# terryye/cuda_FlashAttention

Measured on AMD Instinct MI355X. Metric: FA2 fwd+bwd TFLOP/s at (B=4,H=16,N=8192,d=128); % MFMA peak, higher is better.
Workload: dtype bf16; 1 GPU; FA2 forward+backward bf16, (B=4,H=16,N=8192,d=128) per GPU, non-causal (BASELINE configs[2]); flops = 14 B H N^2 d; B=4, H=16, N=8192, d=128, parallelism=head-sharded replicas x1

## Files before the change

### cuda_flashattention_amd/csrc/fa2_bwd_bf16.hip

```cpp
#include <type_traits>

#include "fa2_regfile.h"
#include "fa2_launch.h"

namespace fa2 {

constexpr float kNoKeyRC = -1.0e30f;
constexpr float kNoKeyLq = 1.0e30f;

template <int D>
__global__ void __launch_bounds__(256) fa2_bwd_delta_kernel(const __bf16* __restrict__ dO,
                                                            const __bf16* __restrict__ O,
                                                            const float* __restrict__ L,
                                                            float* __restrict__ Dv, float* __restrict__ RC,
                                                            size_t rows, int nq, int q_hs, int q_row0, size_t rc_plane,
                                                            float inv_scale)
{
    const size_t r = ((size_t)blockIdx.x * 256 + threadIdx.x) >> 4;
    const int sub = threadIdx.x & 15;
    const size_t head = r / (size_t)nq, i = r % (size_t)nq;
    const size_t row = head * (size_t)q_hs + i;
    const size_t prow = row + (size_t)q_row0;
    float acc = 0.0f;
    if (r < rows) {
#pragma unroll
        for (int c = sub * 8; c < D; c += 128) {
            const bf16x8 a = *reinterpret_cast<const bf16x8*>(dO + row * D + c);
            const bf16x8 b = *reinterpret_cast<const bf16x8*>(O + row * D + c);
#pragma unroll
            for (int e = 0; e < 8; ++e) acc += (float)a[e] * (float)b[e];
        }
    }
#pragma unroll
    for (int off = 8; off >= 1; off >>= 1) acc += __shfl_xor(acc, off, 16);
    if (r < rows && sub == 0) {
        Dv[prow] = acc;
        const float l = L[row];
        RC[prow] = l == -INFINITY ? kNoKeyRC : -l * inv_scale;
        RC[rc_plane + prow] = -acc;
    }
}

__global__ void __launch_bounds__(256) fa2_bwd_dsink_kernel(const float* __restrict__ Dv, const float* __restrict__ L,
                                                            const float* __restrict__ sink, float* __restrict__ dsink,
                                                            int batch, int heads, int nq, int q_hs, int q_row0)
{
    __shared__ float part[256];
    const int h = blockIdx.x, tid = threadIdx.x;
    const float s = sink[h];
    float acc = 0.0f;
    if (s != -INFINITY) {
        for (int b = 0; b < batch; ++b) {
            const size_t row0 = ((size_t)b * heads + h) * (size_t)q_hs;
#pragma unroll 8
            for (int i = tid; i < nq; i += 256)
                acc -= __builtin_amdgcn_exp2f((s - L[row0 + i]) * kLog2e) * Dv[row0 + q_row0 + i];
        }
    }
    part[tid] = acc;
    __syncthreads();
#pragma unroll
    for (int off = 128; off >= 1; off >>= 1) {
        if (tid < off) part[tid] += part[tid + off];
        __syncthreads();
    }
    if (tid == 0) dsink[h] = part[0];
}

static hipError_t launch_dsink(const SinkGrad& sg, const BwdArgs& a, int nq, hipStream_t stream)
{
    if (!sg.sink || !sg.dsink || sg.heads < 1 || a.BH % sg.heads != 0) return hipErrorInvalidValue;
    hipLaunchKernelGGL(fa2_bwd_dsink_kernel, dim3((unsigned)sg.heads), dim3(256), 0, stream, (const float*)a.D, a.L, sg.sink, sg.dsink,
                       a.BH / sg.heads, sg.heads, nq, a.q_hs, a.q_row0);
    return hipGetLastError();
}

constexpr int kBwdRows = 256;
constexpr int kDqWaves = 4;
constexpr int kDqKV = 64;
constexpr int kDkQ = 32;

typedef __attribute__((address_space(3))) void* lptr_t;

#include "fa2_bwd_dq_body.inc"

#define FA2_DQ_CLOBBERS "memory", "vcc", FA2_RF512
#define FA2_DQ_OPS_128 [r0] "v"(roff[0]), [r1] "v"(roff[1]), [r2] "v"(roff[2]), [r3] "v"(roff[3]), [r4] "v"(roff[4]), [r5] "v"(roff[5]), \
    [r6] "v"(roff[6]), [r7] "v"(roff[7]), [t0] "v"(toff[0]), [t1] "v"(toff[1]), [t2] "v"(toff[2]), [t3] "v"(toff[3]), [t4] "v"(toff[4]),     \
    [t5] "v"(toff[5]), [t6] "v"(toff[6]), [t7] "v"(toff[7])
#define FA2_DQ_OPS_64 [r0] "v"(roff[0]), [r1] "v"(roff[1]), [r2] "v"(roff[2]), [r3] "v"(roff[3]), [t0] "v"(toff[0]), [t1] "v"(toff[1]),    \
    [t2] "v"(toff[2]), [t3] "v"(toff[3])
// ... 382 lines not shown
        tile(std::integral_constant<int, 1>{}, t + 1);
    }
    }

    asm volatile("s_waitcnt lgkmcnt(0)" ::: "memory");
    mfma_acc_settle();
    static_for<2>([&](auto KB) {
        constexpr int kb = decltype(KB)::value;
        const int key = kw0 + 32 * kb + ki;
        char* dKk = (char*)p.dK + slab + (size_t)(key < N ? key : 0) * ROWB;
        char* dVk = (char*)p.dV + slab + (size_t)(key < N ? key : 0) * ROWB;
        static_for<4 * DT>([&](auto G) {
            constexpr int dt = decltype(G)::value / 4, g = decltype(G)::value % 4;
            constexpr int RK = A_DK + 16 * (kb * DT + dt) + 4 * g, RV = A_DV + 16 * (kb * DT + dt) + 4 * g;
            bf16x4 a, b;
            a[0] = (__bf16)(aread<RK>() * p.scale); a[1] = (__bf16)(aread<RK + 1>() * p.scale);
            a[2] = (__bf16)(aread<RK + 2>() * p.scale); a[3] = (__bf16)(aread<RK + 3>() * p.scale);
            b[0] = (__bf16)aread<RV>(); b[1] = (__bf16)aread<RV + 1>();
            b[2] = (__bf16)aread<RV + 2>(); b[3] = (__bf16)aread<RV + 3>();
            if (key < N) {
                *reinterpret_cast<bf16x4*>(dKk + 2 * (32 * dt + 8 * g + 4 * h)) = a;
                *reinterpret_cast<bf16x4*>(dVk + 2 * (32 * dt + 8 * g + 4 * h)) = b;
            }
        });
    });
}

template <int D, bool CAUSAL>
__global__ void __launch_bounds__(256, 1) __attribute__((amdgpu_num_vgpr(60))) fa2_bwd_dkdv_kernel(BwdArgs p)
{
    const int ncb = (p.Nk + kDkKeys - 1) / kDkKeys;
    int kvhead, cb;
    map_block(blockIdx.x, p.BH / p.kv_group, ncb, kvhead, cb);
    bwd_dkdv_impl<D, CAUSAL>(p, kvhead, cb);
}

template <int D, bool CAUSAL>
__global__ void __launch_bounds__(256, 1) __attribute__((amdgpu_num_vgpr(60))) fa2_bwd_dkdv_varlen_kernel(VarlenBwdArgs v)
{
    int kvhead, idx;
    map_block(blockIdx.x, v.a.BH / v.a.kv_group, v.n_key_items, kvhead, idx);
    const VarlenItem it = uniform_item(v.key_items, idx);
    bwd_dkdv_impl<D, CAUSAL>(bwd_varlen_view<D>(v.a, it), kvhead, it.block);
}

template <int D, bool CAUSAL>
static hipError_t launch_bwd_one(const BwdArgs& a, hipStream_t stream, const SinkGrad* sg)
{
    const size_t rows = (size_t)a.BH * a.Nq;
    hipError_t e = hipSuccess;
    if (a.phases & 1) {
        hipLaunchKernelGGL((fa2_bwd_delta_kernel<D>), dim3((unsigned)((rows * 16 + 255) / 256)), dim3(256), 0,
                           stream, (const __bf16*)a.dO, (const __bf16*)a.O, a.L, a.D, a.RC, rows, a.Nq, a.q_hs, a.q_row0,
                           (size_t)a.BH * a.q_hs, 1.0f / a.scale);
        e = hipGetLastError();
        if (e != hipSuccess) return e;
        if (sg && (e = launch_dsink(*sg, a, a.Nq, stream)) != hipSuccess) return e;
    }
    const int nb = (a.Nq + kBwdRows - 1) / kBwdRows;
    constexpr int lds_dq = 3 * 2 * kDqKV * D * 2;
    constexpr int lds_dk = kDkKeys * D * 2 + 2 * (2 * 2 * kDkQ * D * 2 + 512);
    if (a.phases & 2) {
        e = launch_lds<fa2_bwd_dq_kernel<D, CAUSAL>>(dim3((unsigned)(nb * a.BH)), dim3(256), lds_dq, stream, a);
        if (e != hipSuccess) return e;
    }
    if (a.phases & 4) {
        const int ncb = (a.Nk + kDkKeys - 1) / kDkKeys;
        e = launch_lds<fa2_bwd_dkdv_kernel<D, CAUSAL>>(dim3((unsigned)(ncb * (a.BH / a.kv_group))), dim3(256), lds_dk, stream, a);
    }
    return e;
}

template <int D, bool CAUSAL>
static hipError_t launch_bwd_varlen_one(const VarlenBwdArgs& v, hipStream_t stream, const SinkGrad* sg)
{
    const BwdArgs& a = v.a;
    const size_t rows = (size_t)a.BH * a.q_hs;
    hipLaunchKernelGGL((fa2_bwd_delta_kernel<D>), dim3((unsigned)((rows * 16 + 255) / 256)), dim3(256), 0, stream,
                       (const __bf16*)a.dO, (const __bf16*)a.O, a.L, a.D, a.RC, rows, a.q_hs, a.q_hs, 0, rows, 1.0f / a.scale);
    hipError_t e = hipGetLastError();
    if (e != hipSuccess) return e;
    if (sg && (e = launch_dsink(*sg, a, a.q_hs, stream)) != hipSuccess) return e;
    constexpr int lds_dq = 3 * 2 * kDqKV * D * 2;
    constexpr int lds_dk = kDkKeys * D * 2 + 2 * (2 * 2 * kDkQ * D * 2 + 512);
    e = launch_lds<fa2_bwd_dq_varlen_kernel<D, CAUSAL>>(dim3((unsigned)(v.n_row_items * a.BH)), dim3(256), lds_dq, stream, v);
    if (e != hipSuccess) return e;
    return launch_lds<fa2_bwd_dkdv_varlen_kernel<D, CAUSAL>>(dim3((unsigned)(v.n_key_items * (a.BH / a.kv_group))), dim3(256), lds_dk,
                                                            stream, v);
}

hipError_t launch_bwd_varlen_bf16(const VarlenBwdArgs& v, hipStream_t stream, const SinkGrad* sg)
{
    const BwdArgs& a = v.a;
    if (a.kv_group < 1 || a.BH % a.kv_group != 0 || v.n_row_items < 1 || v.n_key_items < 1 || !v.row_items || !v.key_items)
        return hipErrorInvalidValue;
    if (a.d == 128) return a.causal ? launch_bwd_varlen_one<128, true>(v, stream, sg) : launch_bwd_varlen_one<128, false>(v, stream, sg);
    if (a.d == 64) return a.causal ? launch_bwd_varlen_one<64, true>(v, stream, sg) : launch_bwd_varlen_one<64, false>(v, stream, sg);
    return hipErrorInvalidValue;
}

hipError_t launch_bwd_bf16(const BwdArgs& a, hipStream_t stream, const SinkGrad* sg)
{
    if (a.kv_group < 1 || a.BH % a.kv_group != 0) return hipErrorInvalidValue;
    if (a.d == 128) return a.causal ? launch_bwd_one<128, true>(a, stream, sg) : launch_bwd_one<128, false>(a, stream, sg);
    if (a.d == 64) return a.causal ? launch_bwd_one<64, true>(a, stream, sg) : launch_bwd_one<64, false>(a, stream, sg);
    return hipErrorInvalidValue;
}

}
```

### cuda_flashattention_amd/csrc/fa2_bwd_fused.hip

```cpp
#include <cstdlib>
#include <cstring>
#include <type_traits>

#include "fa2_regfile.h"
#include "fa2_launch.h"

namespace fa2 {

#include "fa2_bwd_fused_body.inc"

typedef __attribute__((address_space(3))) void* fused_lptr_t;

#ifndef FA2_FUSED_DSKEY
#define FA2_FUSED_DSKEY(row) (((row) >> 1) & 7)
#endif

#ifndef FA2_FUSED_DIAG
#define FA2_FUSED_DIAG 0
#endif

constexpr int kFusedRegFile = RF512;

#define FA2_FUSED_CLOBBERS "memory", "vcc", FA2_RF512
#define FA2_FUSED_OPS_128 [r0] "v"(roff[0]), [r1] "v"(roff[1]), [r2] "v"(roff[2]), [r3] "v"(roff[3]), [r4] "v"(roff[4]), [r5] "v"(roff[5]),  \
// ... 27 lines not shown
    FA2_FUSED_CASE(TAG, DD, 0, 0) FA2_FUSED_CASE(TAG, DD, 0, 1) FA2_FUSED_CASE(TAG, DD, 1, 0) FA2_FUSED_CASE(TAG, DD, 1, 1) FA2_FUSED_CASE(TAG, DD, 2, 0) FA2_FUSED_CASE(TAG, DD, 2, 1)
    FA2_FUSED_CASES(, 128) FA2_FUSED_CASES(64, 64)
#undef FA2_FUSED_CASES
#undef FA2_FUSED_CASE
}

template <int BUF, int PAR, int VMW>
__device__ __forceinline__ void fused_body(const uint32_t (&roff)[8], const uint32_t (&toff)[8], uint32_t rcv, float c2)
{
#define FA2_FUSED_CASE(B, P) \
    if constexpr (BUF == B && PAR == P) asm volatile(FA2_FUSED_BODY_B##B##_P##P : : FA2_FUSED_OPS_128, [vm] "i"(VMW) : FA2_FUSED_CLOBBERS);
    FA2_FUSED_CASE(0, 0) FA2_FUSED_CASE(0, 1) FA2_FUSED_CASE(1, 0) FA2_FUSED_CASE(1, 1) FA2_FUSED_CASE(2, 0) FA2_FUSED_CASE(2, 1)
#undef FA2_FUSED_CASE
}

template <int DQT>
__device__ __forceinline__ void fused_dq_atomic(__amdgpu_buffer_rsrc_t rs, uint32_t voff, uint32_t soff)
{
    asm volatile(
        "s_add_u32 s12, %2, 4096\n\ts_add_u32 s13, %2, 8192\n\ts_add_u32 s14, %2, 12288\n\t"
        "buffer_atomic_add_f32 v%c3, %0, %1, %2 offen\n\tbuffer_atomic_add_f32 v%c4, %0, %1, %2 offen offset:512\n\t"
        "buffer_atomic_add_f32 v%c5, %0, %1, %2 offen offset:1024\n\tbuffer_atomic_add_f32 v%c6, %0, %1, %2 offen offset:1536\n\t"
        "buffer_atomic_add_f32 v%c7, %0, %1, s12 offen\n\tbuffer_atomic_add_f32 v%c8, %0, %1, s12 offen offset:512\n\t"
        "buffer_atomic_add_f32 v%c9, %0, %1, s12 offen offset:1024\n\tbuffer_atomic_add_f32 v%c10, %0, %1, s12 offen offset:1536\n\t"
        "buffer_atomic_add_f32 v%c11, %0, %1, s13 offen\n\tbuffer_atomic_add_f32 v%c12, %0, %1, s13 offen offset:512\n\t"
        "buffer_atomic_add_f32 v%c13, %0, %1, s13 offen offset:1024\n\tbuffer_atomic_add_f32 v%c14, %0, %1, s13 offen offset:1536\n\t"
        "buffer_atomic_add_f32 v%c15, %0, %1, s14 offen\n\tbuffer_atomic_add_f32 v%c16, %0, %1, s14 offen offset:512\n\t"
        "buffer_atomic_add_f32 v%c17, %0, %1, s14 offen offset:1024\n\tbuffer_atomic_add_f32 v%c18, %0, %1, s14 offen offset:1536\n\t"
        "s_nop 1"
        : : "v"(voff), "s"(rs), "s"(soff), "i"(DQT), "i"(DQT + 1), "i"(DQT + 2), "i"(DQT + 3), "i"(DQT + 4), "i"(DQT + 5), "i"(DQT + 6),
            "i"(DQT + 7), "i"(DQT + 8), "i"(DQT + 9), "i"(DQT + 10), "i"(DQT + 11), "i"(DQT + 12), "i"(DQT + 13), "i"(DQT + 14),
            "i"(DQT + 15)
        : "memory", "s12", "s13", "s14", "v255");
}

template <int VF, int KS, int S>
__device__ __forceinline__ void fused_load_vfrag(const char* v0, const char* v1)
{
#ifndef FA2_FUSED_KV_NT
#define FA2_FUSED_KV_NT ""
#define FA2_FUSED_KV_AUX 0
#endif
    asm volatile("global_load_dwordx4 v[%c2:%c3], %0, off offset:%c4" FA2_FUSED_KV_NT "\n\tglobal_load_dwordx4 v[%c5:%c6], %1, off offset:%c4" FA2_FUSED_KV_NT
                 : : "v"(v0), "v"(v1), "i"(VF + 4 * S), "i"(VF + 4 * S + 3), "i"(32 * S), "i"(VF + 4 * (KS + S)), "i"(VF + 4 * (KS + S) + 3)
                 : "memory", "v255");
}

template <int DQT>
__device__ __forceinline__ void fused_dq_zero()
{
    static_for<16>([&](auto R) { vset<kFusedRegFile, CL_TOP, DQT + decltype(R)::value>(0u); });
}

constexpr int kCtlTicket = 0, kCtlNextHead = 32 * 16, kCtlError = 32 * 17, kCtlHeadmap = 32 * 18;
constexpr int kHmPad = 16;
constexpr int kSpinLimit = FA2_FUSED_SPIN_LIMIT;

struct FusedArgs {
    BwdArgs b;
    float* dQacc;
    int* ctl;
    int npad;
    const float* rc;
    int fault;
};

#ifdef FA2_TEST_HOOKS
static int g_hook_fault = 0, g_hook_grid = 0, g_hook_last_grid = 0;
extern "C" void fa2_test_set_fused_hooks(int fault, int grid) { g_hook_fault = fault; g_hook_grid = grid; }
extern "C" int fa2_test_last_fused_grid(void) { return g_hook_last_grid; }
#define FA2_HOOK_NOTE_GRID(n) (g_hook_last_grid = (n))
#else
constexpr int g_hook_fault = 0, g_hook_grid = 0;
#define FA2_HOOK_NOTE_GRID(n) ((void)0)
#endif

__device__ __forceinline__ int fused_ctl_ints(int BH, int ncb) { return kCtlHeadmap + 16 * (BH + kHmPad) + 9 * BH * ncb; }

__device__ __forceinline__ int fused_load_sc1(const int* p)
{
    int v;
    asm volatile("global_load_dword %0, %1, off sc1\n\ts_waitcnt vmcnt(0)" : "=v"(v) : "v"(p) : "memory");
    return v;
}
__device__ __forceinline__ void fused_seen_set(int v)
{
    asm volatile("v_mov_b32 v39, %0" : : "s"(v) : "v39");
}

__device__ __forceinline__ int fused_lane_id() { return (int)__builtin_amdgcn_mbcnt_hi(~0u, __builtin_amdgcn_mbcnt_lo(~0u, 0u)); }
template <int OFF>
__device__ __forceinline__ int fused_mail_read(uint32_t lds_addr)
{
    int v;
    asm volatile("v_mov_b32 %0, %1\n\tds_read_b32 %0, %0 offset:%c2\n\ts_waitcnt lgkmcnt(0)" : "=&v"(v) : "s"(lds_addr), "i"(OFF) : "memory");
    return __builtin_amdgcn_readfirstlane(v);
}

__device__ __forceinline__ void fused_store_flag(int* p, int v)
{
    asm volatile("global_store_dword %0, %1, off" : : "v"(p), "v"(v) : "memory");
}

__device__ __forceinline__ bool fused_spin_over(int* ctl, int spins)
{
    if (spins > kSpinLimit) {
        atomicExch(ctl + kCtlError, 1);
        return true;
    }
    return (spins & 1023) == 0 && fused_load_sc1(ctl + kCtlError) != 0;
}

template <bool CHAIN, bool CAUSAL, bool RAGGED = false, bool RECT = false, int HD = 128>
__global__ void __launch_bounds__(256, 1) __attribute__((amdgpu_num_vgpr(39))) fa2_bwd_fused_kernel(FusedArgs fp)
{
    static_assert(CHAIN || !RAGGED, "the atomics form has no ragged variant");
    static_assert(!RECT || (CHAIN && !CAUSAL && !RAGGED), "rectangular blocks: chained, unmasked, aligned");
    static_assert(HD == 128 || (HD == 64 && CHAIN && !RECT), "head_dim 64: chained, square");
    extern __shared__ __attribute__((aligned(16))) char smem[];
    const BwdArgs& p = fp.b;
    constexpr int D = HD, ROWB = 2 * D, KS = D / 16, DT = D / 32;
    constexpr int DQW = 128;
    constexpr int TROWS = 32;
    constexpr bool W = D == 128;
    constexpr int QRING = W ? FA2_FUSED_QRING : FA2_FUSED64_QRING, BUFB = W ? FA2_FUSED_BUFB : FA2_FUSED64_BUFB,
                  DSB = W ? FA2_FUSED_DSB : FA2_FUSED64_DSB, LDSB = W ? FA2_FUSED_LDS : FA2_FUSED64_LDS;
    constexpr int CPR = D / 8, RPI = 64 / CPR, NINS = TROWS / RPI;
    constexpr int VF = W ? FA2_FUSED_VF : FA2_FUSED64_VF, DQT = W ? FA2_FUSED_DQT : FA2_FUSED64_DQT,
                  ROFFK = W ? FA2_FUSED_ROFFK : FA2_FUSED64_ROFFK, DSWR = W ? FA2_FUSED_DSWR : FA2_FUSED64_DSWR,
                  DSRD = W ? FA2_FUSED_DSRD : FA2_FUSED64_DSRD, KT = W ? FA2_FUSED_KT : FA2_FUSED64_KT;
    constexpr int VMW = CHAIN ? (W ? 4 : 2) : 63;
    int* const mail = reinterpret_cast<int*>(smem + LDSB);
    const uint32_t mail_addr = __builtin_amdgcn_readfirstlane((uint32_t)(uintptr_t)smem) + LDSB;

    const int tid = threadIdx.x;
    const int lane = tid & 63;
    const int wave = __builtin_amdgcn_readfirstlane(tid >> 6);
    const int ki = lane & 31;
    const int h = lane >> 5;
    const int N = p.Nk;
    const int NP = RAGGED ? fp.npad : N;
    const int NQ = RECT ? p.Nq : N;
    const int NPQ = RECT ? NQ : NP;
    const int QHS = RECT ? p.q_hs : N, KHS = RECT ? p.k_hs : N;
    const int QR0 = RECT ? p.q_row0 : 0;
    const int ncb = NP / 256;
    const int ntiles = NPQ / TROWS;
    const int niter = ((ntiles + 1 + 5) / 6) * 6;
    const float c2 = p.scale * kLog2e;
    const size_t rc_plane = (size_t)p.BH * (RECT ? QHS : NP);

    const uint32_t lbase = (uint32_t)(uintptr_t)smem;
    const int trq = (lane & 15) >> 2, trp = lane & 3, trcb = (lane >> 4) & 1;
    uint32_t roff[KS], toff[2 * DT];
#pragma unroll
    for (int s = 0; s < KS; ++s) roff[s] = lbase + QRING + lds_off<D>(ki, 2 * s + h);
#pragma unroll
    for (int dt = 0; dt < DT; ++dt)
#pragma unroll
        for (int jj = 0; jj < 2; ++jj)
            toff[2 * dt + jj] = lbase + QRING + lds_off<D>(8 * jj + 4 * h + trq, 4 * dt + 2 * trcb + (trp >> 1)) + 8 * (trp & 1);
    const uint32_t rcv = lbase + QRING + 2 * TROWS * ROWB + 16 * h;
    static_for<KS>([&](auto S) {
        constexpr int sidx = decltype(S)::value;
        vset<kFusedRegFile, CL_TOP, ROFFK + sidx>(lbase + lds_off<D>(ki + 64 * wave, 2 * sidx + h));
    });
    const int ecol = W ? wave : (wave & 1), ekey0 = W ? 0 : 128 * (wave >> 1);
    static_for<2>([&](auto JJ) {
        constexpr int jj = decltype(JJ)::value;
        vset<kFusedRegFile, CL_TOP, KT + jj>(lbase + ekey0 * ROWB + lds_off<D>(8 * jj + 4 * h + trq, 4 * ecol + 2 * trcb + (trp >> 1)) + 8 * (trp & 1));
        const int row = 8 * jj + 4 * h + trq;
        vset<kFusedRegFile, CL_TOP, DSRD + jj>(lbase + DSB + (ekey0 + row) * 64 + 8 * ((4 * trcb + trp) ^ FA2_FUSED_DSKEY(row)));
    });
    static_for<4>([&](auto C) {
        constexpr int c = decltype(C)::value;
        vset<kFusedRegFile, CL_TOP, DSWR + c>(lbase + DSB + (64 * wave + ki) * 64 + 8 * (((2 * c) | h) ^ FA2_FUSED_DSKEY(ki)));
    });
    const int doff = lds_dma_off<D>(wave * RPI, lane);
    const uint32_t dqv = CHAIN ? (uint32_t)(wave * 4096 + lane * 16) : (uint32_t)(((4 * h) * D + 32 * wave + ki) * 4);
    const auto rc_rsrc = __builtin_amdgcn_make_buffer_rsrc((void*)fp.rc, 0, (int)(2 * rc_plane * 4), 0x00020000);

    int xcc = 0;
    if constexpr (CHAIN) {
        asm volatile("s_getreg_b32 %0, hwreg(HW_REG_XCC_ID, 0, 4)" : "=s"(xcc));
    }
    int* const prog_base = fp.ctl + kCtlHeadmap + 16 * (p.BH + kHmPad);
#ifndef FA2_FUSED_CAUSAL_G
#define FA2_FUSED_CAUSAL_G 2
#endif
    const int G = CAUSAL ? max(1, min(FA2_FUSED_CAUSAL_G, p.BH / 8)) : 1;
    const auto ctl_rsrc = __builtin_amdgcn_make_buffer_rsrc((void*)fp.ctl, 0, CHAIN ? fused_ctl_ints(p.BH, ncb) * 4 : 0, 0x00020000);

    auto take_ticket = [&]() {
        if (wave == 0 && fused_lane_id() == 0) {
            int hd, j = 0;
            do {
                const int u = atomicAdd(fp.ctl + kCtlTicket + 32 * xcc, 1);
                const int r = u % (G * ncb);
                const int k = (u / (G * ncb)) * G + r % G;
                j = r / G;
                hd = -2;
                if (k < p.BH + kHmPad) {
                    int* hm = fp.ctl + kCtlHeadmap + xcc * (p.BH + kHmPad) + k;
                    int v = 0, spins = 0;
                    if (j == 0) {
                        if (k > 0)
                            while ((v = fused_load_sc1(hm - 1)) == 0)
                                if (fused_spin_over(fp.ctl, ++spins)) break;
                        if (k > 0 && v == 0) {
                            v = -1;
                        } else {
                            const int g = atomicAdd(fp.ctl + kCtlNextHead, 1);
                            v = g < p.BH ? g + 1 : -1;
                        }
                        fused_store_flag(hm, v);
                    } else {
                        while ((v = fused_load_sc1(hm)) == 0)
                            if (fused_spin_over(fp.ctl, ++spins)) { v = -1; break; }
                    }
                    hd = v > 0 ? v - 1 : (r % G == 0 ? -2 : -1);
                }
            } while (hd == -1);
            mail[0] = hd;
            mail[1] = j;
            mail[2] = hd >= 0 ? fused_load_sc1(fp.ctl + kCtlError) : 0;
        }
    };
    auto issue_unit_loads = [&](int head_, int cb_) {
        const size_t slab_ = (size_t)(head_ / p.kv_group) * KHS * ROWB;
        const char* Kh_ = (const char*)p.K + slab_;
        const char* Vh_ = (const char*)p.V + slab_;
        const int kw0_ = cb_ * 256 + wave * 64;
        const int lane_u = (int)__builtin_amdgcn_mbcnt_hi(~0u, __builtin_amdgcn_mbcnt_lo(~0u, 0u));
        const int vk0 = RAGGED ? min(kw0_ + (lane_u & 31), N - 1) : kw0_ + (lane_u & 31);
        const int vk1 = RAGGED ? min(kw0_ + 32 + (lane_u & 31), N - 1) : kw0_ + 32 + (lane_u & 31);
        const char* v0 = Vh_ + (size_t)vk0 * ROWB + 16 * (lane_u >> 5);
        const char* v1 = Vh_ + (size_t)vk1 * ROWB + 16 * (lane_u >> 5);
        static_for<KS>([&](auto S) { fused_load_vfrag<VF, KS, decltype(S)::value>(v0, v1); });
        const auto k_rsrc = __builtin_amdgcn_make_buffer_rsrc((void*)Kh_, 0, N * ROWB, 0x00020000);
#pragma unroll
        for (int j = wave; j < 256 / RPI; j += 4)
            __builtin_amdgcn_raw_ptr_buffer_load_lds(k_rsrc, (fused_lptr_t)(smem + j * 1024), 16, doff, (cb_ * 256 + j * RPI) * ROWB, 0, FA2_FUSED_KV_AUX);
    };

    auto next_unit_loads = [&]() {
        if constexpr (CHAIN) {
            take_ticket();
            __syncthreads();
            const int hn = fused_mail_read<0>(mail_addr);
            if (hn >= 0) issue_unit_loads(hn, fused_mail_read<4>(mail_addr));
        }
    };
    next_unit_loads();

    for (;;) {
#ifdef FA2_FUSED_STATS
        const uint64_t s_pull = __builtin_readcyclecounter();
#endif
        int head, cb, err0 = 0;
        if constexpr (CHAIN) {
            head = fused_mail_read<0>(mail_addr);
            cb = fused_mail_read<4>(mail_addr);
            err0 = fused_mail_read<8>(mail_addr);
            if (head < 0) break;
        } else {
            map_block(blockIdx.x, p.BH, ncb, head, cb);
            issue_unit_loads(head, cb);
        }
        const size_t slab = (size_t)head * QHS * ROWB;
        const char* Qh = (const char*)p.Q + slab;
        const char* Gh = (const char*)p.dO + slab;
        const int kw0 = cb * 256 + wave * 64;
        {
            const u32x4 z = {0u, 0u, 0u, 0u};
            static_for<4 * DT>([&](auto T) { azero16<kFusedRegFile, CL_ACC, 16 * decltype(T)::value>(z); });
        }

        const auto q_rsrc = __builtin_amdgcn_make_buffer_rsrc((void*)Qh, 0, NQ * ROWB, 0x00020000);
        const auto g_rsrc = __builtin_amdgcn_make_buffer_rsrc((void*)Gh, 0, NQ * ROWB, 0x00020000);
        const int rcoff = (int)(((wave == 0 ? 0 : rc_plane) + (size_t)head * (RECT ? QHS : NP) + QR0 + (fused_lane_id() & 31)) * 4);
        auto stage = [&](int t, int buf) {
            char* b = smem + QRING + buf * BUFB;
#pragma unroll
            for (int j = wave; j < 2 * NINS; j += 4) {
                const int which = j / NINS, piece = j % NINS;
                const int soff = (t * TROWS + piece * RPI) * ROWB;
                __builtin_amdgcn_raw_ptr_buffer_load_lds(which ? g_rsrc : q_rsrc, (fused_lptr_t)(b + which * (TROWS * ROWB) + piece * 1024),
                                                         16, doff, soff, 0, 0);
            }
            if (wave < 2 && fused_lane_id() < 32)
                __builtin_amdgcn_raw_ptr_buffer_load_lds(rc_rsrc, (fused_lptr_t)(b + 2 * TROWS * ROWB + wave * 128), 4, rcoff, t * TROWS * 4, 0, 0);
        };
        const int n_u = CAUSAL ? ntiles - 8 * cb : ntiles;
        const int niter_u = CAUSAL ? ((n_u + 1 + 5) / 6) * 6 : niter;
        const bool ragged_unit = RAGGED && !CAUSAL && cb == ncb - 1;
        const int first_masked = CAUSAL ? ((n_u - 8) / 6) * 6 : (ragged_unit ? 0 : niter_u);
        auto tl = [&](int u) { return CAUSAL ? ntiles - 1 - u : u; };
        stage(tl(0), 0);
#ifdef FA2_FUSED_PREFILL
        stage(tl(1), 1);
        stage(tl(2), 2);
#endif
        fused_dq_zero<DQT>();
        asm volatile("s_waitcnt vmcnt(0)" ::: "memory");
        __syncthreads();
        if constexpr (W) asm volatile(FA2_FUSED_PRO : : FA2_FUSED_OPS_128, [vm] "i"(VMW) : FA2_FUSED_CLOBBERS);
        else asm volatile(FA2_FUSED64_PRO : : FA2_FUSED_OPS_64, [vm] "i"(VMW) : FA2_FUSED_CLOBBERS);

        const auto dq_rsrc = __builtin_amdgcn_make_buffer_rsrc((void*)(fp.dQacc + (size_t)head * NPQ * DQW), 0, NPQ * DQW * 4, 0x00020000);
        int* const mine = prog_base + head * ncb + cb;
        const int* const prev = mine - 1;
        const int prev_off = (int)((prev - fp.ctl) * 4);
        const int mine_off = (int)((mine - fp.ctl) * 4);
        if constexpr (CHAIN) fused_seen_set(0);
        int err = err0;
#ifdef FA2_FUSED_STATS
        int st_steps = 0, st_polls = 0, st_cycles = 0;
        const uint64_t u0 = __builtin_readcyclecounter();
#endif

        const auto null_rsrc = __builtin_amdgcn_make_buffer_rsrc((void*)fp.dQacc, 0, 0, 0x00020000);
        const bool hp_unit = cb > 0;
        const auto lrs_unit = hp_unit && !(FA2_FUSED_DIAG & 2) ? dq_rsrc : null_rsrc;
        auto step = [&](auto BUF, auto PAR, auto MASKED, auto FAST_, int t) {
            constexpr int buf = decltype(BUF)::value, par = decltype(PAR)::value;
            constexpr bool masked = decltype(MASKED)::value;
            constexpr bool FAST = decltype(FAST_)::value;
            if constexpr (CHAIN && FAST) {
                FusedStep f;
                f.drs = dq_rsrc;
                f.lrs = lrs_unit;
                f.dso = (uint32_t)(tl(t - 1) * TROWS * DQW * 4);
                f.lso = (uint32_t)(tl(t) * TROWS * DQW * 4);
                f.qrs = q_rsrc; f.grs = g_rsrc; f.rcrs = rc_rsrc; f.ctl = ctl_rsrc;
                f.qso = (uint32_t)(tl(t + 1) * TROWS * ROWB + wave * 1024);
                f.rcso = (uint32_t)(tl(t + 1) * TROWS * 4);
                f.pvo = (uint32_t)prev_off; f.mso = (uint32_t)mine_off;
                f.need = (hp_unit && !err && !(FA2_FUSED_DIAG & 1)) ? t + 1 : (int)0x80000000;
                f.pval = t;
#ifdef FA2_TEST_HOOKS
                if (fp.fault && cb == 1) f.pval = 0;
#endif
                fused_cbody<D, buf, par, VMW, false>(roff, toff, rcv, c2, dqv, (uint32_t)doff, (uint32_t)rcoff, lbase + QRING + wave * 1024,
                                                  lbase + QRING + wave * 128, wave, f, err, 0, 0);
            } else if constexpr (CHAIN) {
                FusedStep f;
                const bool live = t >= 1 && t <= n_u;
                const bool more = t + 1 < n_u;
                const bool has_prev = t < n_u && cb > 0;
                f.drs = live ? dq_rsrc : null_rsrc;
// ... 208 lines not shown
    if (hipGetDevice(&dev) != hipSuccess || dev < 0 || dev >= 64) { if (why) *why = "no current device"; return false; }
    if (!verdict[dev]) {
        hipDeviceProp_t pr;
        if (hipGetDeviceProperties(&pr, dev) != hipSuccess) { if (why) *why = "device properties unavailable"; return false; }
        verdict[dev] = strncmp(pr.gcnArchName, "gfx950", 6) != 0 ? 2 : pr.multiProcessorCount != 256 ? 3 : 1;
    }
    static const char* const text[] = {"", "single five-product kernel (gfx950, 256 CUs: the layout the ordered hand-off was validated on)",
                                       "two kernels: device is not gfx950", "two kernels: device does not expose 256 CUs (partitioned GPU): "
                                       "the ordered hand-off was validated in SPX mode only"};
    if (why) *why = text[verdict[dev]];
    return verdict[dev] == 1;
}

hipError_t bwd_fused_read_error(const int* ctl, int* err, hipStream_t stream)
{
    hipError_t e = hipMemcpyAsync(err, ctl + kCtlError, sizeof(int), hipMemcpyDeviceToHost, stream);
    if (e != hipSuccess) return e;
    return hipStreamSynchronize(stream);
}

hipError_t bwd_fused_clear_error(int* ctl, hipStream_t stream)
{
    return launch_fill_f32(reinterpret_cast<float*>(ctl + kCtlError), 1, 0.0f, stream);
}

size_t bwd_fused_kvpart_bytes(int BH, int N, int d) { return (size_t)2 * BH * N * d * 2; }
size_t bwd_fused_ctl_bytes(int BH, int N) { return (size_t)(kCtlHeadmap + 16 * (BH + kHmPad) + 9 * BH * ((N + 255) / 256)) * sizeof(int); }

template <int HD>
static hipError_t launch_chained_square(bool causal, bool ragged, dim3 grid, int lds, hipStream_t stream, const FusedArgs& fa)
{
    if (causal)
        return ragged ? launch_lds<fa2_bwd_fused_kernel<true, true, true, false, HD>>(grid, dim3(256), lds, stream, fa)
                      : launch_lds<fa2_bwd_fused_kernel<true, true, false, false, HD>>(grid, dim3(256), lds, stream, fa);
    return ragged ? launch_lds<fa2_bwd_fused_kernel<true, false, true, false, HD>>(grid, dim3(256), lds, stream, fa)
                  : launch_lds<fa2_bwd_fused_kernel<true, false, false, false, HD>>(grid, dim3(256), lds, stream, fa);
}

hipError_t launch_bwd_fused_bf16(const BwdArgs& a, float* dQacc, int* ctl, int mode, hipStream_t stream, float* rcpad, void* kvpart,
                                 const SinkGrad* sg)
{
    const int npad = (a.Nk + 255) / 256 * 256;
    const bool ragged = npad != a.Nk;
    const bool rect = a.Nq != a.Nk || a.q_hs != a.Nq || a.k_hs != a.Nk || a.q_row0 != 0;
    if ((a.d != 128 && a.d != 64) || a.Nk < 1 || a.Nq < 1) return hipErrorInvalidValue;
    if (a.d == 64 && (mode != 1 || rect)) return hipErrorInvalidValue;
    if (rect && (mode != 1 || a.causal || ragged || a.Nq % 32 != 0 || a.q_row0 < 0 || a.q_hs < a.q_row0 + a.Nq || a.k_hs < a.Nk))
        return hipErrorInvalidValue;
    if (ragged && (mode != 1 || !rcpad)) return hipErrorInvalidValue;
    const bool grouped = a.kv_group > 1;
    if (a.kv_group < 1 || a.BH % a.kv_group != 0 || (grouped && (mode != 1 || rect || !kvpart))) return hipErrorInvalidValue;
    if (a.causal && (mode != 1 || a.causal_shift != 0)) return hipErrorInvalidValue;
    hipError_t e = hipSuccess;
    if (a.phases & 1) {
        BwdArgs d = a;
        d.phases = 1;
        e = launch_bwd_bf16(d, stream, sg);
        if (e != hipSuccess) return e;
    }
    if (!(a.phases & 8)) return hipSuccess;
    const size_t elems = (size_t)a.BH * (rect ? a.Nq : npad) * 128;
    const int units = a.BH * (npad / 256);
    if (ragged) {
        const size_t n = (size_t)2 * a.BH * npad;
        hipLaunchKernelGGL(fa2_bwd_fused_rcpad_kernel, dim3((unsigned)((n + 255) / 256)), dim3(256), 0, stream, (const float*)a.RC, rcpad,
                           a.BH, a.Nk, npad);
        e = hipGetLastError();
        if (e != hipSuccess) return e;
    }
    FusedArgs fa{a, dQacc, ctl, npad, ragged ? (const float*)rcpad : (const float*)a.RC, g_hook_fault};
    const size_t part_elems = (size_t)a.BH * a.Nk * a.d;
    if (grouped) {
        fa.b.dK = kvpart;
        fa.b.dV = (__bf16*)kvpart + part_elems;
    }
    const int lds = (a.d == 64 ? FA2_FUSED64_LDS : FA2_FUSED_LDS) + 16;
    if (mode == 0) {
        e = launch_fill_f32(dQacc, elems, 0.0f, stream);
        if (e != hipSuccess) return e;
        e = bwd_fused_clear_error(ctl, stream);
        if (e != hipSuccess) return e;
        e = launch_lds<fa2_bwd_fused_kernel<false, false>>(dim3((unsigned)units), dim3(256), lds, stream, fa);
    } else {
        static int cus[64] = {};
        int dev = 0;
        e = hipGetDevice(&dev);
        if (e != hipSuccess) return e;
        if (dev < 0 || dev >= 64) return hipErrorInvalidDevice;
        if (!cus[dev]) {
            e = hipDeviceGetAttribute(&cus[dev], hipDeviceAttributeMultiprocessorCount, dev);
            if (e != hipSuccess) return e;
        }
        e = launch_fill_f32(reinterpret_cast<float*>(ctl), bwd_fused_ctl_bytes(a.BH, a.Nk) / sizeof(float), 0.0f, stream);
        if (e != hipSuccess) return e;
        int avail = cus[dev] - (a.reserve_cus > 0 ? a.reserve_cus : 0);
        if (avail < 1) avail = 1;
        int wgs = units < avail ? units : avail;
        if (g_hook_grid >= 1 && g_hook_grid < wgs) wgs = g_hook_grid;
        FA2_HOOK_NOTE_GRID(wgs);
        const dim3 grid((unsigned)wgs);
        if (rect)
            e = launch_lds<fa2_bwd_fused_kernel<true, false, false, true>>(grid, dim3(256), lds, stream, fa);
        else
            e = a.d == 64 ? launch_chained_square<64>(a.causal, ragged, grid, lds, stream, fa)
                          : launch_chained_square<128>(a.causal, ragged, grid, lds, stream, fa);
    }
    if (e != hipSuccess) return e;
    if (mode == 0)
        hipLaunchKernelGGL(fa2_bwd_fused_dq_out_kernel, dim3(2048), dim3(256), 0, stream, dQacc, (__bf16*)a.dQ, elems / 8, a.scale,
                           (const int*)nullptr);
    else if (a.d == 64)
        hipLaunchKernelGGL(fa2_bwd_fused_dq_out_chain64_kernel, dim3(4096), dim3(256), 0, stream, dQacc, (__bf16*)a.dQ, elems / 8, a.scale,
                           ctl + kCtlError, a.Nk, npad);
    else
        hipLaunchKernelGGL(fa2_bwd_fused_dq_out_chain_kernel, dim3(4096), dim3(256), 0, stream, dQacc, (__bf16*)a.dQ, elems / 4, a.scale,
                           ctl + kCtlError, rect ? a.Nq : a.Nk, rect ? a.Nq : npad, rect ? a.q_hs : a.Nk);
    e = hipGetLastError();
    if (e != hipSuccess || !grouped) return e;
    hipLaunchKernelGGL(fa2_bwd_fused_dkdv_out_kernel, dim3(4096), dim3(256), 0, stream, (const bf16x8*)fa.b.dK, (const bf16x8*)fa.b.dV,
                       (bf16x8*)a.dK, (bf16x8*)a.dV, (size_t)a.Nk * a.d / 8, (size_t)(a.BH / a.kv_group), a.kv_group);
    return hipGetLastError();
}

}
```

### cuda_flashattention_amd/csrc/fa2_launch.h

```cpp
#pragma once
#include <hip/hip_runtime.h>
#include <stddef.h>

namespace fa2 {

struct FwdArgs {
    const void* Q;
    const void* K;
    const void* V;
    void* O;
    float* L;
    float* Oacc;
    float* M;
    int BH, Nq, Nk, d;
    float scale;
    int causal;
    int causal_shift;
    int resume;
    int finalize;
    int q_hs, k_hs;
    int kv_group;
    const float* sink;
    int sink_heads;
};

hipError_t launch_fwd1_bf16(const FwdArgs& a, hipStream_t stream);

struct VarlenItem {
    int q_row0, k_row0;
    int len_q, len_k;
    int block;
};
struct VarlenFwdArgs { FwdArgs a; const VarlenItem* items; int n_items; };
hipError_t launch_fwd1_varlen_bf16(const VarlenFwdArgs& v, hipStream_t stream);
hipError_t launch_accumulate_bf16(float* acc, const void* src, size_t rows, size_t cols, size_t pitch, int init, hipStream_t stream);
hipError_t launch_finalize_state(const float* Oacc, const float* M, float* L, void* O, size_t rows, int d, hipStream_t stream);

struct FwdFp8Args {
    const void* Q; const void* K; const void* V;
    void* Vt;
    float* kn;
    void* O;
    float* L;
    int BH, N, Npad, d;
    float scale;
    int causal;
    float o_scale;
};
hipError_t launch_fwd_fp8(const FwdFp8Args& a, hipStream_t stream);

struct BwdArgs {
    const void* Q; const void* K; const void* V; const void* O; const void* dO;
    const float* L;
    void* dQ; void* dK; void* dV;
    float* D;
    float* RC;
    int BH, Nq, Nk, d;
    int q_hs, k_hs;
    int q_row0;
    float scale;
    int causal;
    int causal_shift;
    int phases;
    int reserve_cus;
    int kv_group;
};

struct SinkGrad { const float* sink; float* dsink; int heads; };

hipError_t launch_bwd_bf16(const BwdArgs& a, hipStream_t stream, const SinkGrad* sg = nullptr);
struct VarlenBwdArgs {
    BwdArgs a;
    const VarlenItem* row_items; const VarlenItem* key_items;
    int n_row_items, n_key_items;
};
hipError_t launch_bwd_varlen_bf16(const VarlenBwdArgs& v, hipStream_t stream, const SinkGrad* sg = nullptr);
size_t bwd_fused_ctl_bytes(int BH, int N);
size_t bwd_fused_kvpart_bytes(int BH, int N, int d);
hipError_t launch_bwd_fused_bf16(const BwdArgs& a, float* dQacc, int* ctl, int mode, hipStream_t stream, float* rcpad = nullptr,
                                 void* kvpart = nullptr, const SinkGrad* sg = nullptr);
bool bwd_fused_device_ok(const char** why);
hipError_t bwd_fused_read_error(const int* ctl, int* err, hipStream_t stream);
hipError_t bwd_fused_clear_error(int* ctl, hipStream_t stream);

struct F32Args {
    const float* Q; const float* K; const float* V; float* O; float* L;
    const float* dO; float* dQ; float* dK; float* dV; float* D;
    int BH, N, d;
    float scale;
    int causal;
    int phases;
    int Nk;
    float* M;
    int resume, finalize;
};
hipError_t launch_fwd_f32(const F32Args& a, hipStream_t stream);
hipError_t launch_bwd_f32(const F32Args& a, hipStream_t stream);

template <auto K, typename A>
inline hipError_t launch_lds(dim3 grid, dim3 block, int lds, hipStream_t stream, const A& arg)
{
    static bool done[64] = {};
    int dev = 0;
    hipError_t e = hipGetDevice(&dev);
    if (e != hipSuccess) return e;
    if (dev < 0 || dev >= 64) return hipErrorInvalidDevice;
    if (!done[dev]) {
        e = hipFuncSetAttribute(reinterpret_cast<const void*>(K), hipFuncAttributeMaxDynamicSharedMemorySize, lds);
        if (e != hipSuccess) return e;
        done[dev] = true;
    }
    hipLaunchKernelGGL(K, grid, block, lds, stream, arg);
    return hipGetLastError();
}

hipError_t launch_fa1_f32(const float* Q, const float* K, const float* V, float* O, float* l, float* m, int N, int d, int Bc,
                          hipStream_t stream);

hipError_t launch_fill_f32(float* p, size_t n, float value, hipStream_t stream);
hipError_t launch_mfma_probe(const void* in, float* out, int iters, int blocks, hipStream_t stream);
hipError_t launch_f32_to_bf16(const float* src, void* dst, size_t n, hipStream_t stream);
hipError_t launch_bf16_to_f32(const void* src, float* dst, size_t n, hipStream_t stream);
hipError_t launch_read_clocks(unsigned long long* out, hipStream_t stream);
// ... 3 lines not shown
```

Before: 1280 TFLOP/s.

## Fold backward delta preprocessing into the fused backward kernel for late heads

The standalone delta kernel now runs only over the first eight heads and also zeroes the control buffer, which removes the separate fill launch. The remaining heads' delta/RC rows are computed inside the fused backward kernel as 256-row chunks, handed out through an atomic ticket. Early units take chunks under a time quota, and units reaching a late head drain the rest and spin until all chunks finish. This aims to hide the preprocessing pass and a launch behind compute, at the cost of LDS ring reuse, extra synchronisation and per-unit recomputation of lane operands.

```diff
diff --git a/cuda_flashattention_amd/csrc/fa2_bwd_bf16.hip b/cuda_flashattention_amd/csrc/fa2_bwd_bf16.hip
--- a/cuda_flashattention_amd/csrc/fa2_bwd_bf16.hip
+++ b/cuda_flashattention_amd/csrc/fa2_bwd_bf16.hip
@@ -5,7 +5,6 @@
 
 namespace fa2 {
 
-constexpr float kNoKeyRC = -1.0e30f;
 constexpr float kNoKeyLq = 1.0e30f;
 
 template <int D>
@@ -14,8 +13,9 @@
                                                             const float* __restrict__ L,
                                                             float* __restrict__ Dv, float* __restrict__ RC,
                                                             size_t rows, int nq, int q_hs, int q_row0, size_t rc_plane,
-                                                            float inv_scale)
-{
+                                                            float inv_scale, int* __restrict__ zero, size_t nzero)
+{
+    for (size_t z = (size_t)blockIdx.x * 256 + threadIdx.x; z < nzero; z += (size_t)gridDim.x * 256) zero[z] = 0;
     const size_t r = ((size_t)blockIdx.x * 256 + threadIdx.x) >> 4;
     const int sub = threadIdx.x & 15;
     const size_t head = r / (size_t)nq, i = r % (size_t)nq;
@@ -27,16 +27,13 @@
         for (int c = sub * 8; c < D; c += 128) {
             const bf16x8 a = *reinterpret_cast<const bf16x8*>(dO + row * D + c);
             const bf16x8 b = *reinterpret_cast<const bf16x8*>(O + row * D + c);
-#pragma unroll
-            for (int e = 0; e < 8; ++e) acc += (float)a[e] * (float)b[e];
+            acc = bwd_delta_dot8(acc, a, b);
         }
     }
-#pragma unroll
-    for (int off = 8; off >= 1; off >>= 1) acc += __shfl_xor(acc, off, 16);
+    acc = bwd_delta_tree16(acc);
     if (r < rows && sub == 0) {
         Dv[prow] = acc;
-        const float l = L[row];
-        RC[prow] = l == -INFINITY ? kNoKeyRC : -l * inv_scale;
+        RC[prow] = bwd_delta_rc0(L[row], inv_scale);
         RC[rc_plane + prow] = -acc;
     }
 }
@@ -525,7 +522,7 @@
     if (a.phases & 1) {
         hipLaunchKernelGGL((fa2_bwd_delta_kernel<D>), dim3((unsigned)((rows * 16 + 255) / 256)), dim3(256), 0,
                            stream, (const __bf16*)a.dO, (const __bf16*)a.O, a.L, a.D, a.RC, rows, a.Nq, a.q_hs, a.q_row0,
-                           (size_t)a.BH * a.q_hs, 1.0f / a.scale);
+                           (size_t)a.BH * a.q_hs, 1.0f / a.scale, (int*)nullptr, (size_t)0);
         e = hipGetLastError();
         if (e != hipSuccess) return e;
         if (sg && (e = launch_dsink(*sg, a, a.Nq, stream)) != hipSuccess) return e;
@@ -550,7 +547,8 @@
     const BwdArgs& a = v.a;
     const size_t rows = (size_t)a.BH * a.q_hs;
     hipLaunchKernelGGL((fa2_bwd_delta_kernel<D>), dim3((unsigned)((rows * 16 + 255) / 256)), dim3(256), 0, stream,
-                       (const __bf16*)a.dO, (const __bf16*)a.O, a.L, a.D, a.RC, rows, a.q_hs, a.q_hs, 0, rows, 1.0f / a.scale);
+                       (const __bf16*)a.dO, (const __bf16*)a.O, a.L, a.D, a.RC, rows, a.q_hs, a.q_hs, 0, rows, 1.0f / a.scale,
+                       (int*)nullptr, (size_t)0);
     hipError_t e = hipGetLastError();
     if (e != hipSuccess) return e;
     if (sg && (e = launch_dsink(*sg, a, a.q_hs, stream)) != hipSuccess) return e;
@@ -572,6 +570,16 @@
     return hipErrorInvalidValue;
 }
 
+hipError_t launch_bwd_delta_heads(const BwdArgs& a, int heads, int* zero, size_t nzero, hipStream_t stream)
+{
+    if (a.d != 128 || heads < 1 || heads > a.BH || a.Nq != a.q_hs || a.q_row0 != 0) return hipErrorInvalidValue;
+    const size_t rows = (size_t)heads * a.Nq;
+    hipLaunchKernelGGL((fa2_bwd_delta_kernel<128>), dim3((unsigned)((rows * 16 + 255) / 256)), dim3(256), 0, stream,
+                       (const __bf16*)a.dO, (const __bf16*)a.O, a.L, a.D, a.RC, rows, a.Nq, a.q_hs, 0, (size_t)a.BH * a.q_hs,
+                       1.0f / a.scale, zero, nzero);
+    return hipGetLastError();
+}
+
 hipError_t launch_bwd_bf16(const BwdArgs& a, hipStream_t stream, const SinkGrad* sg)
 {
     if (a.kv_group < 1 || a.BH % a.kv_group != 0) return hipErrorInvalidValue;
diff --git a/cuda_flashattention_amd/csrc/fa2_bwd_fused.hip b/cuda_flashattention_amd/csrc/fa2_bwd_fused.hip
--- a/cuda_flashattention_amd/csrc/fa2_bwd_fused.hip
+++ b/cuda_flashattention_amd/csrc/fa2_bwd_fused.hip
@@ -103,7 +103,8 @@
     static_for<16>([&](auto R) { vset<kFusedRegFile, CL_TOP, DQT + decltype(R)::value>(0u); });
 }
 
-constexpr int kCtlTicket = 0, kCtlNextHead = 32 * 16, kCtlError = 32 * 17, kCtlHeadmap = 32 * 18;
+constexpr int kCtlTicket = 0, kCtlNextHead = 32 * 16, kCtlError = 32 * 17, kCtlChunk = 32 * 18, kCtlChunksDone = 32 * 19,
+              kCtlHeadmap = 32 * 20;
 constexpr int kHmPad = 16;
 constexpr int kSpinLimit = FA2_FUSED_SPIN_LIMIT;
 
@@ -114,6 +115,10 @@
     int npad;
     const float* rc;
     int fault;
+    int dk;
+    int h0;
+    int nchunks;
+    float inv_scale;
 };
 
 #ifdef FA2_TEST_HOOKS
@@ -174,6 +179,7 @@
     constexpr int DQW = 128;
     constexpr int TROWS = 32;
     constexpr bool W = D == 128;
+    constexpr bool DKOK = CHAIN && !CAUSAL && !RAGGED && !RECT && HD == 128;
     constexpr int QRING = W ? FA2_FUSED_QRING : FA2_FUSED64_QRING, BUFB = W ? FA2_FUSED_BUFB : FA2_FUSED64_BUFB,
                   DSB = W ? FA2_FUSED_DSB : FA2_FUSED64_DSB, LDSB = W ? FA2_FUSED_LDS : FA2_FUSED64_LDS;
     constexpr int CPR = D / 8, RPI = 64 / CPR, NINS = TROWS / RPI;
@@ -203,15 +209,22 @@
 
     const uint32_t lbase = (uint32_t)(uintptr_t)smem;
     const int trq = (lane & 15) >> 2, trp = lane & 3, trcb = (lane >> 4) & 1;
-    uint32_t roff[KS], toff[2 * DT];
-#pragma unroll
-    for (int s = 0; s < KS; ++s) roff[s] = lbase + QRING + lds_off<D>(ki, 2 * s + h);
-#pragma unroll
-    for (int dt = 0; dt < DT; ++dt)
-#pragma unroll
-        for (int jj = 0; jj < 2; ++jj)
-            toff[2 * dt + jj] = lbase + QRING + lds_off<D>(8 * jj + 4 * h + trq, 4 * dt + 2 * trcb + (trp >> 1)) + 8 * (trp & 1);
-    const uint32_t rcv = lbase + QRING + 2 * TROWS * ROWB + 16 * h;
+    uint32_t roff[KS], toff[2 * DT], rcv, dqv;
+    int doff;
+    auto lane_operands = [&](int ln) {
+        const int ki_ = ln & 31, h_ = ln >> 5, trq_ = (ln & 15) >> 2, trp_ = ln & 3, trcb_ = (ln >> 4) & 1;
+#pragma unroll
+        for (int s = 0; s < KS; ++s) roff[s] = lbase + QRING + lds_off<D>(ki_, 2 * s + h_);
+#pragma unroll
+        for (int dt = 0; dt < DT; ++dt)
+#pragma unroll
+            for (int jj = 0; jj < 2; ++jj)
+                toff[2 * dt + jj] = lbase + QRING + lds_off<D>(8 * jj + 4 * h_ + trq_, 4 * dt + 2 * trcb_ + (trp_ >> 1)) + 8 * (trp_ & 1);
+        rcv = lbase + QRING + 2 * TROWS * ROWB + 16 * h_;
+        doff = lds_dma_off<D>(wave * RPI, ln);
+        dqv = CHAIN ? (uint32_t)(wave * 4096 + ln * 16) : (uint32_t)(((4 * h_) * D + 32 * wave + ki_) * 4);
+    };
+    if constexpr (!DKOK) lane_operands(lane);
     static_for<KS>([&](auto S) {
         constexpr int sidx = decltype(S)::value;
         vset<kFusedRegFile, CL_TOP, ROFFK + sidx>(lbase + lds_off<D>(ki + 64 * wave, 2 * sidx + h));
@@ -227,8 +240,6 @@
         constexpr int c = decltype(C)::value;
         vset<kFusedRegFile, CL_TOP, DSWR + c>(lbase + DSB + (64 * wave + ki) * 64 + 8 * (((2 * c) | h) ^ FA2_FUSED_DSKEY(ki)));
     });
-    const int doff = lds_dma_off<D>(wave * RPI, lane);
-    const uint32_t dqv = CHAIN ? (uint32_t)(wave * 4096 + lane * 16) : (uint32_t)(((4 * h) * D + 32 * wave + ki) * 4);
     const auto rc_rsrc = __builtin_amdgcn_make_buffer_rsrc((void*)fp.rc, 0, (int)(2 * rc_plane * 4), 0x00020000);
 
     int xcc = 0;
@@ -289,9 +300,10 @@
         const char* v1 = Vh_ + (size_t)vk1 * ROWB + 16 * (lane_u >> 5);
         static_for<KS>([&](auto S) { fused_load_vfrag<VF, KS, decltype(S)::value>(v0, v1); });
         const auto k_rsrc = __builtin_amdgcn_make_buffer_rsrc((void*)Kh_, 0, N * ROWB, 0x00020000);
+        const int doff_u = DKOK ? lds_dma_off<D>(wave * RPI, lane_u) : doff;
 #pragma unroll
         for (int j = wave; j < 256 / RPI; j += 4)
-            __builtin_amdgcn_raw_ptr_buffer_load_lds(k_rsrc, (fused_lptr_t)(smem + j * 1024), 16, doff, (cb_ * 256 + j * RPI) * ROWB, 0, FA2_FUSED_KV_AUX);
+            __builtin_amdgcn_raw_ptr_buffer_load_lds(k_rsrc, (fused_lptr_t)(smem + j * 1024), 16, doff_u, (cb_ * 256 + j * RPI) * ROWB, 0, FA2_FUSED_KV_AUX);
     };
 
     auto next_unit_loads = [&]() {
@@ -303,6 +315,87 @@
         }
     };
     next_unit_loads();
+
+#ifndef FA2_FUSED_DK_QUOTA
+#define FA2_FUSED_DK_QUOTA 300
+#endif
+#ifndef FA2_FUSED_DK_CHUNK0
+#define FA2_FUSED_DK_CHUNK0 400
+#endif
+    constexpr int kDkRing = 5, kDkGroups = 8, kDkWaveB = kDkRing * 4096;
+    static_assert(!DKOK || QRING + 4 * kDkWaveB <= LDSB, "the chunk ring lives in the Q / dO ring and the dS tiles");
+    auto dk_chunk = [&](int c) {
+        int lane_c = fused_lane_id();
+        asm volatile("" : "+v"(lane_c));
+        const size_t row0 = (size_t)fp.h0 * N + (size_t)c * 256 + wave * 64;
+        const auto g_rs = __builtin_amdgcn_make_buffer_rsrc((void*)((const char*)p.dO + row0 * ROWB), 0, 64 * ROWB, 0x00020000);
+        const auto o_rs = __builtin_amdgcn_make_buffer_rsrc((void*)((const char*)p.O + row0 * ROWB), 0, 64 * ROWB, 0x00020000);
+        char* const ring = smem + QRING + wave * kDkWaveB;
+        const uint32_t rd = lbase + QRING + wave * kDkWaveB + lane_c * 16;
+        auto issue = [&](auto J) {
+            constexpr int j = decltype(J)::value, slot = (j % kDkRing) * 4096;
+#pragma unroll
+            for (int pp = 0; pp < 2; ++pp) {
+                __builtin_amdgcn_raw_ptr_buffer_load_lds(g_rs, (fused_lptr_t)(ring + slot + pp * 2048), 16, lane_c * 16, (8 * j + 4 * pp) * ROWB, 0, 0);
+                __builtin_amdgcn_raw_ptr_buffer_load_lds(o_rs, (fused_lptr_t)(ring + slot + pp * 2048 + 1024), 16, lane_c * 16, (8 * j + 4 * pp) * ROWB, 0, 0);
+            }
+        };
+        static_for<kDkRing>([&](auto J) { issue(J); });
+        float res = 0.0f;
+        static_for<kDkGroups>([&](auto J) {
+            constexpr int j = decltype(J)::value, slot = (j % kDkRing) * 4096;
+            constexpr int newer = (j + kDkRing < kDkGroups ? kDkRing : kDkGroups - j) - 1;
+            asm volatile("s_waitcnt vmcnt(%c0)" : : "i"(4 * newer) : "memory");
+#pragma unroll
+            for (int pp = 0; pp < 2; ++pp) {
+                u32x4 a, b;
+                asm volatile("ds_read_b128 %0, %2 offset:%c3\n\tds_read_b128 %1, %2 offset:%c4\n\ts_waitcnt lgkmcnt(0)"
+                             : "=&v"(a), "=&v"(b) : "v"(rd), "i"(slot + pp * 2048), "i"(slot + pp * 2048 + 1024) : "memory");
+                const float s = bwd_delta_tree16(bwd_delta_dot8(0.0f, __builtin_bit_cast(bf16x8, a), __builtin_bit_cast(bf16x8, b)));
+                const float mine = __shfl(s, (lane_c & 3) * 16);
+                if ((lane_c >> 2) == 2 * j + pp) res = mine;
+            }
+            if constexpr (j + kDkRing < kDkGroups) issue(std::integral_constant<int, j + kDkRing>{});
+        });
+        const float rc0 = bwd_delta_rc0(p.L[row0 + lane_c], fp.inv_scale);
+        asm volatile("global_store_dword %0, %1, %2 sc1" : : "v"(lane_c * 4), "v"(res), "s"(p.D + row0) : "memory");
+        asm volatile("global_store_dword %0, %1, %2 sc1" : : "v"(lane_c * 4), "v"(rc0), "s"(p.RC + row0) : "memory");
+        asm volatile("global_store_dword %0, %1, %2 sc1" : : "v"(lane_c * 4), "v"(-res), "s"(p.RC + rc_plane + row0) : "memory");
+        asm volatile("s_waitcnt vmcnt(0)" ::: "memory");
+        __syncthreads();
+        if (wave == 0 && lane_c == 0) __hip_atomic_fetch_add(fp.ctl + kCtlChunksDone, 1, __ATOMIC_RELAXED, __HIP_MEMORY_SCOPE_AGENT);
+    };
+    auto dk_chunks = [&](long long ticks, uint64_t t0) {
+        uint64_t last = FA2_FUSED_DK_CHUNK0;
+        for (;;) {
+            const uint64_t t1 = __builtin_amdgcn_s_memrealtime();
+            if (wave == 0 && fused_lane_id() == 0) {
+                int c = -1;
+                if (ticks < 0 || (long long)(t1 - t0 + last) <= ticks) {
+                    c = atomicAdd(fp.ctl + kCtlChunk, 1);
+                    if (c >= fp.nchunks) c = -1;
+                }
+                mail[3] = c;
+            }
+            __syncthreads();
+            const int c = fused_mail_read<12>(mail_addr);
+            if (c < 0) break;
+            dk_chunk(c);
+            last = __builtin_amdgcn_s_memrealtime() - t1;
+        }
+    };
+    auto dk_wait_all = [&]() {
+        if (wave == 0) {
+            int spins = 0;
+            while (fused_load_sc1(fp.ctl + kCtlChunksDone) < fp.nchunks)
+                if (fused_spin_over(fp.ctl, ++spins)) break;
+            __builtin_amdgcn_fence(__ATOMIC_ACQUIRE, "agent");
+            asm volatile("s_waitcnt vmcnt(0)" ::: "memory");
+        }
+        __syncthreads();
+    };
+    bool dk_pending = DKOK && fp.dk != 0;
+    bool dk_first = true;
 
     for (;;) {
 #ifdef FA2_FUSED_STATS
@@ -339,14 +432,34 @@
                 __builtin_amdgcn_raw_ptr_buffer_load_lds(which ? g_rsrc : q_rsrc, (fused_lptr_t)(b + which * (TROWS * ROWB) + piece * 1024),
                                                          16, doff, soff, 0, 0);
             }
-            if (wave < 2 && fused_lane_id() < 32)
-                __builtin_amdgcn_raw_ptr_buffer_load_lds(rc_rsrc, (fused_lptr_t)(b + 2 * TROWS * ROWB + wave * 128), 4, rcoff, t * TROWS * 4, 0, 0);
+            if (wave < 2 && fused_lane_id() < 32) {
+                if (DKOK && fp.dk)
+                    __builtin_amdgcn_raw_ptr_buffer_load_lds(rc_rsrc, (fused_lptr_t)(b + 2 * TROWS * ROWB + wave * 128), 4, rcoff, t * TROWS * 4, 0, 16);
+                else
+                    __builtin_amdgcn_raw_ptr_buffer_load_lds(rc_rsrc, (fused_lptr_t)(b + 2 * TROWS * ROWB + wave * 128), 4, rcoff, t * TROWS * 4, 0, 0);
+            }
         };
         const int n_u = CAUSAL ? ntiles - 8 * cb : ntiles;
         const int niter_u = CAUSAL ? ((n_u + 1 + 5) / 6) * 6 : niter;
         const bool ragged_unit = RAGGED && !CAUSAL && cb == ncb - 1;
         const int first_masked = CAUSAL ? ((n_u - 8) / 6) * 6 : (ragged_unit ? 0 : niter_u);
         auto tl = [&](int u) { return CAUSAL ? ntiles - 1 - u : u; };
+        if constexpr (DKOK) {
+            const bool late = head >= fp.h0;
+            if (dk_pending && (late || (dk_first && FA2_FUSED_DK_QUOTA > 0))) {
+                dk_chunks(late ? -1 : (long long)cb * FA2_FUSED_DK_QUOTA, __builtin_amdgcn_s_memrealtime());
+                if (late) {
+                    dk_wait_all();
+                    dk_pending = false;
+                }
+            }
+            dk_first = false;
+        }
+        if constexpr (DKOK) {
+            int ln = fused_lane_id();
+            asm volatile("" : "+v"(ln));
+            lane_operands(ln);
+        }
         stage(tl(0), 0);
 #ifdef FA2_FUSED_PREFILL
         stage(tl(1), 1);
@@ -661,7 +774,12 @@
     if (a.kv_group < 1 || a.BH % a.kv_group != 0 || (grouped && (mode != 1 || rect || !kvpart))) return hipErrorInvalidValue;
     if (a.causal && (mode != 1 || a.causal_shift != 0)) return hipErrorInvalidValue;
     hipError_t e = hipSuccess;
-    if (a.phases & 1) {
+    const int h0 = a.BH < 8 ? a.BH : 8;
+    const bool dk = mode == 1 && (a.phases & 9) == 9 && a.d == 128 && !rect && !ragged && !a.causal && !grouped && !sg && a.BH > h0;
+    if (dk) {
+        e = launch_bwd_delta_heads(a, h0, ctl, bwd_fused_ctl_bytes(a.BH, a.Nk) / sizeof(int), stream);
+        if (e != hipSuccess) return e;
+    } else if (a.phases & 1) {
         BwdArgs d = a;
         d.phases = 1;
         e = launch_bwd_bf16(d, stream, sg);
@@ -678,6 +796,10 @@
         if (e != hipSuccess) return e;
     }
     FusedArgs fa{a, dQacc, ctl, npad, ragged ? (const float*)rcpad : (const float*)a.RC, g_hook_fault};
+    fa.dk = dk;
+    fa.h0 = h0;
+    fa.nchunks = dk ? (a.BH - h0) * (npad / 256) : 0;
+    fa.inv_scale = 1.0f / a.scale;
     const size_t part_elems = (size_t)a.BH * a.Nk * a.d;
     if (grouped) {
         fa.b.dK = kvpart;
@@ -700,7 +822,7 @@
             e = hipDeviceGetAttribute(&cus[dev], hipDeviceAttributeMultiprocessorCount, dev);
             if (e != hipSuccess) return e;
         }
-        e = launch_fill_f32(reinterpret_cast<float*>(ctl), bwd_fused_ctl_bytes(a.BH, a.Nk) / sizeof(float), 0.0f, stream);
+        if (!dk) e = launch_fill_f32(reinterpret_cast<float*>(ctl), bwd_fused_ctl_bytes(a.BH, a.Nk) / sizeof(float), 0.0f, stream);
         if (e != hipSuccess) return e;
         int avail = cus[dev] - (a.reserve_cus > 0 ? a.reserve_cus : 0);
         if (avail < 1) avail = 1;
diff --git a/cuda_flashattention_amd/csrc/fa2_launch.h b/cuda_flashattention_amd/csrc/fa2_launch.h
--- a/cuda_flashattention_amd/csrc/fa2_launch.h
+++ b/cuda_flashattention_amd/csrc/fa2_launch.h
@@ -69,6 +69,25 @@
 struct SinkGrad { const float* sink; float* dsink; int heads; };
 
 hipError_t launch_bwd_bf16(const BwdArgs& a, hipStream_t stream, const SinkGrad* sg = nullptr);
+hipError_t launch_bwd_delta_heads(const BwdArgs& a, int heads, int* zero, size_t nzero, hipStream_t stream);
+
+#ifdef __HIPCC__
+constexpr float kNoKeyRC = -1.0e30f;
+template <typename V8>
+__device__ __forceinline__ float bwd_delta_dot8(float acc, const V8& a, const V8& b)
+{
+#pragma unroll
+    for (int e = 0; e < 8; ++e) acc += (float)a[e] * (float)b[e];
+    return acc;
+}
+__device__ __forceinline__ float bwd_delta_tree16(float acc)
+{
+#pragma unroll
+    for (int off = 8; off >= 1; off >>= 1) acc += __shfl_xor(acc, off, 16);
+    return acc;
+}
+__device__ __forceinline__ float bwd_delta_rc0(float l, float inv_scale) { return l == -INFINITY ? kNoKeyRC : -l * inv_scale; }
+#endif
 struct VarlenBwdArgs {
     BwdArgs a;
     const VarlenItem* row_items; const VarlenItem* key_items;
```

Result: no change. 1285 TFLOP/s (median of 6 runs) (+0.4%).
